# lllllcf/Realtime-Depth-Estimation-Nconv

Hardware: AMD Instinct MI355X
Metric: frames/sec (352x1216 sparse depth, DNET NConv U-Net forward, B=8 per GPU) (higher is better)
Workload: dtype fp32

## Files before the change

### realtime-depth-estimation-nconv_amd/csrc/nconv_fwd_head.hip

```cpp
#include "nconv_prologue.h"

namespace nconv {

namespace {

constexpr int kHT = 256, kHTH = 16, kHTW = 32;
constexpr int kSH = kHTH + 8, kSW = kHTW + 8;
constexpr int kHH = kHTH + 4, kHW = kHTW + 4;
constexpr int kHP = kHW - 16;
constexpr int kHPlane = kHH * kHP;
constexpr int kHPS = kHPlane + 1;
constexpr int kFrag = 2 * 3 * 64 * 4;
constexpr int kLut = 0, kW8R = 4096, kW8C = kW8R + kSH * kSW, kTabEnd = kW8C + kHTH * kSW;
constexpr int kDP = 8 * 64 + 16;
constexpr int kDOff = (kTabEnd + 15) & ~15;

typedef const float __attribute__((address_space(4))) cfloat;
typedef __bf16 bf16x8 __attribute__((ext_vector_type(8)));

template <bool TR>
__global__ __launch_bounds__(kHT) __attribute__((amdgpu_waves_per_eu(5, 8))) void fwd_head_exact(LayerDev d2, TailArgs t, float* __restrict__ y,
                                                      float* __restrict__ yc) {
    const nconv_layer& L = d2.L;
    __shared__ __attribute__((aligned(16))) float sx[kSH * kSW];
    __shared__ __attribute__((aligned(16))) f2 hp[8 * kHPS];
    __shared__ __attribute__((aligned(16))) float w1t[25 * 8];
    __shared__ unsigned long long rowmask[kSH];
    __shared__ unsigned long long c0row[kSH];
    __shared__ unsigned c0col[kSW];
    __shared__ int tile_nan;
    static_assert(kDOff + 8 * kDP * 4 <= (int)sizeof(hp), "D2 tables and transpose fit the plane region");
    const int tid = threadIdx.x;
    const int H = L.Ho, W = L.Wo;
    const TileCoord tc = xcd_tile((W + kHTW - 1) / kHTW, (H + kHTH - 1) / kHTH, L.B);
    const int b = tc.b, R0 = tc.ty * kHTH, C0 = tc.tx * kHTW;
    const bool interior = R0 >= 2 && R0 + kHTH + 2 <= H && C0 >= 2 && C0 + kHTW + 2 <= W;

    if (tid < kSH) rowmask[tid] = c0row[tid] = 0ull;
    if (tid < kSW) c0col[tid] = 0u;
    if (tid == 0) tile_nan = 0;
    if (tid < 200) w1t[tid] = t.w1[(tid & 7) * 25 + (tid >> 3)];
    __syncthreads();
    {
        const __amdgpu_buffer_rsrc_t rs = plane_rsrc(t.s_in + (size_t)b * H * W, H * W * 4);
        constexpr int NE = (kSH * kSW + kHT - 1) / kHT;
        float sv[NE];
#pragma unroll
        for (int k = 0; k < NE; ++k) {
            const int e = tid + kHT * k, r = e / kSW, c = e - (e / kSW) * kSW;
            const int gr = R0 - 4 + r, gc = C0 - 4 + c;
            const bool in = e < kSH * kSW && (unsigned)gr < (unsigned)H && (unsigned)gc < (unsigned)W;
            sv[k] = ld_f32(rs, in ? (unsigned)(gr * W + gc) * 4u : 0x80000000u);
        }
#pragma unroll
        for (int k = 0; k < NE; ++k) {
            const int e = tid + kHT * k, r = e / kSW, c = e - (e / kSW) * kSW;
            if (e < kSH * kSW) {
                const float c0 = sv[k] > t.thresh1 ? 1.0f : 0.0f;
                const float xc = sv[k] * c0;
                sx[e] = xc;
                if (!(xc == 0.f && c0 == 0.f)) atomicOr(&rowmask[r], 1ull << c);
                if (xc != xc) tile_nan = 1;
                if (c0 != 0.f) {
                    atomicOr(&c0row[r], 1ull << c);
                    atomicOr(&c0col[c], 1u << r);
                }
            }
        }
    }
    __syncthreads();

    const int ty = tid >> 4, j = tid & 15;
    f2 accN[8], accD[8];
#pragma unroll
    for (int o = 0; o < 8; ++o) accN[o] = accD[o] = (f2){0.f, 0.f};

    constexpr int NH = (kHH * kHW + kHT - 1) / kHT;
    auto nconv1_pass = [&](bool want_c, auto exact_c0) __attribute__((always_inline)) {
#pragma unroll 1
        for (int k = 0; k < NH; ++k) {
            const int e = tid + kHT * k;
            const int r = e / kHW, c = e - (e / kHW) * kHW;
            const int gr = R0 - 2 + r, gc = C0 - 2 + c;
            const bool valid = e < kHH * kHW;
            const bool in = valid && (unsigned)gr < (unsigned)H && (unsigned)gc < (unsigned)W;
            unsigned m = 0;
#ifndef NCONV_HEAD_PROBE_NO_N1
#pragma unroll
            for (int kh = 0; kh < 5; ++kh) m |= (unsigned)((rowmask[(valid ? r : 0) + kh] >> c) & 31ull) << (5 * kh);
#endif
            m = in ? m : 0u;
            const float* const sxb = sx + r * kSW + c;
            f2 acc[8];
            {
                const bool any = m != 0u;
                const int tp = any ? __builtin_ctz(m) : 0;
                m &= m - 1u;
                const int kh = (tp * 13) >> 6;
                const float xr = sxb[kh * (kSW - 5) + tp];
                const float xc = any ? xr : 0.f;
                const float cv = decltype(exact_c0)::value ? (xc > t.thresh1 ? 1.0f : 0.0f) : 1.0f;
                const f2 v = (f2){xc, any ? cv : 0.f};
                const f4 wa = reinterpret_cast<const f4*>(w1t)[tp * 2], wb = reinterpret_cast<const f4*>(w1t)[tp * 2 + 1];
                const float wv[8] = {wa.x, wa.y, wa.z, wa.w, wb.x, wb.y, wb.z, wb.w};
#pragma unroll
                for (int o = 0; o < 8; ++o) acc[o] = __builtin_elementwise_fma((f2){wv[o], wv[o]}, v, (f2){0.f, 0.f});
            }
            while (m) {
                const int tp = __builtin_ctz(m);
                m &= m - 1;
                const int kh = (tp * 13) >> 6;
                const float xc = sxb[kh * (kSW - 5) + tp];
                const f2 v = (f2){xc, decltype(exact_c0)::value ? (xc > t.thresh1 ? 1.0f : 0.0f) : 1.0f};
                const f4 wa = reinterpret_cast<const f4*>(w1t)[tp * 2], wb = reinterpret_cast<const f4*>(w1t)[tp * 2 + 1];
                const float wv[8] = {wa.x, wa.y, wa.z, wa.w, wb.x, wb.y, wb.z, wb.w};
#pragma unroll
                for (int o = 0; o < 8; ++o) acc[o] = __builtin_elementwise_fma((f2){wv[o], wv[o]}, v, acc[o]);
            }
            const int h0 = (valid && c < kHP) ? (r * kHP + c) * 2 : kHPlane * 2;
            const int h1 = (valid && c >= 16) ? (r * kHP + c - 16) * 2 + 1 : kHPlane * 2 + 1;
            float* const p0 = reinterpret_cast<float*>(hp) + h0;
            float* const p1 = reinterpret_cast<float*>(hp) + h1;
            const unsigned own = (TR && !want_c && in && (unsigned)(r - 2) < (unsigned)kHTH &&
                                  (unsigned)(c - 2) < (unsigned)kHTW) ? (unsigned)(gr * W + gc) * 4u : 0x80000000u;
#pragma unroll
            for (int o = 0; o < 8; ++o) {
                float y1, cc1;
                nconv_epilogue(acc[o].x, acc[o].y, t.eps1, t.b1[o], t.s1[o], y1, cc1);
                if constexpr (TR) {
                    const size_t po1 = ((size_t)b * 8 + o) * H * W;
                    st_f32(plane_rsrc(t.y1 + po1, H * W * 4), own, y1);
                    st_f32(plane_rsrc(t.c1 + po1, H * W * 4), own, cc1);
                }
                const float v = want_c ? cc1 : y1 * cc1;
                p0[o * kHPS * 2] = v;
                p1[o * kHPS * 2] = v;
            }
        }
    };
    auto nconv1_planes = [&](bool want_c) __attribute__((always_inline)) {
        if (tile_nan) nconv1_pass(want_c, std::true_type{});
        else nconv1_pass(want_c, std::false_type{});
    };
    nconv1_planes(false);
    __syncthreads();

    const cfloat* w2t = (const cfloat*)L.waux + kFrag;
    auto sum_planes = [&](f2 (&acc)[8]) __attribute__((always_inline)) {
#pragma unroll 1
        for (int ci = 0; ci < 8; ++ci) {
            const f2* row = hp + ci * kHPS + ty * kHP + j;
            const cfloat* wr = w2t + ci * 200;
#pragma unroll 1
            for (int kh = 0; kh < 5; ++kh, row += kHP, wr += 40) {
                f2 v[5];
#pragma unroll
                for (int kw = 0; kw < 5; ++kw) v[kw] = row[kw];
#pragma unroll
                for (int kw = 0; kw < 5; ++kw)
#pragma unroll
                    for (int o = 0; o < 8; ++o) {
                        const float wv = wr[kw * 8 + o];
                        acc[o] = __builtin_elementwise_fma((f2){wv, wv}, v[kw], acc[o]);
                    }
            }
        }
    };
#ifndef NCONV_HEAD_PROBE_NO_N2
    sum_planes(accN);
#endif
    __syncthreads();
    if (!interior) {
        nconv1_planes(true);
        __syncthreads();
        sum_planes(accD);
    } else {
        unsigned char* const tb = reinterpret_cast<unsigned char*>(hp);
        float* const dt = reinterpret_cast<float*>(tb + kDOff);
        {
            unsigned dq[4];
#pragma unroll
            for (int i = 0; i < 4; ++i)
                dq[i] = ((tid >> (2 * i)) & 1u) * 0x3F80u + ((tid >> (2 * i + 1)) & 1u) * 0x3F800000u;
            reinterpret_cast<uint4*>(tb + kLut)[tid] = make_uint4(dq[0], dq[1], dq[2], dq[3]);
        }
        for (int e = tid; e < kSH * kSW; e += kHT) {
            const int r = e / kSW, c = e - r * kSW;
            tb[kW8R + e] = (unsigned char)(c0row[r] >> c);
            if (r < kHTH) tb[kW8C + e] = c < kHTW ? (unsigned char)(c0col[c + 8] >> r) : 0;
        }
        __syncthreads();
        {
            const int lane = tid & 63, g = lane >> 4, n = lane & 15, w = tid >> 6;
            const uint4* fr = reinterpret_cast<const uint4*>(L.waux) + lane;
            bf16x8 A[2][3];
#pragma unroll
            for (int bb = 0; bb < 2; ++bb)
#pragma unroll
                for (int ks = 0; ks < 3; ++ks) A[bb][ks] = __builtin_bit_cast(bf16x8, fr[(bb * 3 + ks) * 64]);
            const int pb = w * 4 * kSW + n;
            const int o0 = kW8R + g * kSW + pb, o1 = kW8R + (4 + g) * kSW + pb;
            const int o2 = g == 0 ? kW8R + 8 * kSW + pb : (g == 1 ? kW8C + pb : kW8R + 8 * kSW + 8 + pb);
#pragma unroll
            for (int nb = 0; nb < 8; ++nb) {
                const int po = (nb >> 1) * kSW + 16 * (nb & 1);
                const bf16x8 B0 = __builtin_bit_cast(bf16x8, reinterpret_cast<const uint4*>(tb + kLut)[tb[o0 + po]]);
                const bf16x8 B1 = __builtin_bit_cast(bf16x8, reinterpret_cast<const uint4*>(tb + kLut)[tb[o1 + po]]);
                const bf16x8 B2 = __builtin_bit_cast(bf16x8, reinterpret_cast<const uint4*>(tb + kLut)[tb[o2 + po]]);
#pragma unroll
                for (int bb = 0; bb < 2; ++bb) {
                    f4 acc = (f4){0.f, 0.f, 0.f, 0.f};
                    acc = __builtin_amdgcn_mfma_f32_16x16x32_bf16(A[bb][0], B0, acc, 0, 0, 0);
                    acc = __builtin_amdgcn_mfma_f32_16x16x32_bf16(A[bb][1], B1, acc, 0, 0, 0);
                    acc = __builtin_amdgcn_mfma_f32_16x16x32_bf16(A[bb][2], B2, acc, 0, 0, 0);
                    dt[(4 * bb + g) * kDP + (4 * w + (nb >> 1)) * kHTW + 16 * (nb & 1) + n] =
                        (acc.x + acc.y) + acc.z;
                }
            }
        }
        __syncthreads();
#pragma unroll
        for (int o = 0; o < 8; ++o) accD[o] = (f2){dt[o * kDP + ty * kHTW + j], dt[o * kDP + ty * kHTW + j + 16]};
    }

    constexpr unsigned OOB = 0x80000000u;
    const int oh = R0 + ty;
    const size_t plane = (size_t)H * W;
    const int pbytes = (int)(plane * 4);
    const int Hp = H >> 1, Wp = W >> 1;
    const size_t pplane = (size_t)Hp * Wp;
    const int ppbytes = (int)(pplane * 4);
    unsigned so[2], po[2], pcy[2], pcc[2];
    const bool pool_col = ((j & 1) == 0) && (oh >> 1) < Hp;
#pragma unroll
    for (int h = 0; h < 2; ++h) {
        const int ow = C0 + j + 16 * h;
        so[h] = (oh < H && ow < W) ? (unsigned)(oh * W + ow) * 4u : OOB;
        const unsigned pp = (pool_col && (ow >> 1) < Wp) ? (unsigned)((oh >> 1) * Wp + (ow >> 1)) * 4u : OOB;
        po[h] = (ty & 1) == 0 ? pp : OOB;
        pcy[h] = po[h];
        pcc[h] = (ty & 1) ? pp : OOB;
    }
#pragma unroll
    for (int o = 0; o < 8; ++o) {
        float yv[2], cv[2];
        const float s = L.wsum[o], bo = L.bias[o];
#pragma unroll
        for (int h = 0; h < 2; ++h) {
            const float N = h ? accN[o].y : accN[o].x, D = h ? accD[o].y : accD[o].x;
            nconv_epilogue(N, D, L.eps, bo, s, yv[h], cv[h]);
        }
        const size_t ofs = ((size_t)b * 8 + o) * plane;
        const __amdgpu_buffer_rsrc_t ry = plane_rsrc(y + ofs, pbytes), rc = plane_rsrc(yc + ofs, pbytes);
        const size_t pofs = ((size_t)b * 8 + o) * pplane;
        const __amdgpu_buffer_rsrc_t rpy = plane_rsrc(t.py + pofs, ppbytes), rpc = plane_rsrc(t.pc + pofs, ppbytes);
#pragma unroll
        for (int h = 0; h < 2; ++h) {
            st_f32(ry, so[h], yv[h]);
            st_f32(rc, so[h], cv[h]);
#ifdef NCONV_HEAD_PROBE_NO_POOL
            continue;
#endif
            if constexpr (TR) {
                const float yb = shfl_xor16(yv[h]), cb = shfl_xor16(cv[h]);
                const float ya = shfl_xor1(yv[h]), yd = shfl_xor1(yb), ca = shfl_xor1(cv[h]), cd = shfl_xor1(cb);
                int ay, ac;
                st_f32(rpy, po[h], pool4(yv[h], ya, yb, yd, ay));
                st_f32(rpc, po[h], pool4(cv[h], ca, cb, cd, ac));
                st_f32(plane_rsrc((const float*)(t.parg + pofs), ppbytes), po[h],
                       __builtin_bit_cast(float, (unsigned)(ay | (ac << 2))));
            } else {
                const float vm = pair_rows_max(yv[h], cv[h]);
                const float pm = __builtin_elementwise_maximum(vm, shfl_xor1(vm));
                st_f32(rpy, pcy[h], pm);
                st_f32(rpc, pcc[h], pm);
            }
        }
    }
}

__device__ __forceinline__ int frag_slot(int o, int part, int chunk, int j) {
    const int row = 4 * (o & 3) + part, ks = chunk >> 2, g = chunk & 3;
    return (((o >> 2) * 3 + ks) * 64 + g * 16 + row) * 8 + j;
}

constexpr int kHeadUnits = 83;
__device__ __forceinline__ void head_weights_unit(const float* __restrict__ w1, float s1i,
                                                  const float* __restrict__ w2, float* __restrict__ out,
                                                  int blk, int lane) {
    unsigned short* const fb = reinterpret_cast<unsigned short*>(out);
    if (blk == 81) {
        for (int e = lane; e < 1600; e += 64) {
            const int o = e & 7, kk = (e >> 3) % 25, ci = e / 200;
            out[kFrag + e] = w2[(o * 8 + ci) * 25 + kk];
        }
        return;
    }
    if (blk == 82) {
        for (int e = lane; e < kFrag * 2; e += 64) {
            const int j = e & 7, l = (e >> 3) & 63, ks = (e >> 9) % 3;
            const int part = l & 3, chunk = 4 * ks + (l >> 4);
            if (part == 3 || chunk == 11 || (chunk == 10 && j != 0)) fb[e] = 0;
        }
        return;
    }
    const int qh = blk / 9, qw = blk % 9, o = lane >> 3, i = lane & 7;
    double si = 0.0;
#pragma unroll
    for (int kh = 0; kh < 5; ++kh) {
        const int kh1 = qh - kh;
#pragma unroll
        for (int kw = 0; kw < 5; ++kw) {
            const int kw1 = qw - kw;
            const bool v = kh1 >= 0 && kh1 <= 4 && kw1 >= 0 && kw1 <= 4;
            const double a = (double)w2[((o * 8 + i) * 5 + kh) * 5 + kw];
            const double b = (double)w1[v ? (i * 5 + kh1) * 5 + kw1 : 0];
            si = v ? __builtin_fma(a, b, si) : si;
        }
    }
    si /= (double)s1i;
#pragma unroll
    for (int m = 1; m < 8; m <<= 1) si += __shfl_xor(si, m);
    if (i == 0) {
        const float w = (float)si;
        const float hi = __uint_as_float(__float_as_uint(w) & 0xFFFF0000u);
        const float r = w - hi;
        const float mid = __uint_as_float(__float_as_uint(r) & 0xFFFF0000u);
        const float lo = r - mid;
        const int chunk = qw < 8 ? qh : (qh < 8 ? 9 : 10);
        const int j = qw < 8 ? qw : (qh < 8 ? qh : 0);
        fb[frag_slot(o, 0, chunk, j)] = (unsigned short)(__float_as_uint(hi) >> 16);
        fb[frag_slot(o, 1, chunk, j)] = (unsigned short)(__float_as_uint(mid) >> 16);
        fb[frag_slot(o, 2, chunk, j)] = (unsigned short)(__float_as_uint(lo) >> 16);
    }
}

__global__ __launch_bounds__(64) void head_weights(const float* __restrict__ w1, const float* __restrict__ s1,
                                                   const float* __restrict__ w2, float* __restrict__ out) {
    head_weights_unit(w1, s1[threadIdx.x & 7], w2, out, blockIdx.x, threadIdx.x);
}

__global__ __launch_bounds__(kPrepThreads) void weight_prologue(PrepArgs prep, int nprep, const float* __restrict__ w1,
                                                                 const float* __restrict__ w2, float* __restrict__ w21,
                                                                 PhaseArgs ph, int nphase) {
    const int nhead = w21 ? (kHeadUnits + 3) / 4 : 0;
    int blk = blockIdx.x;
    if (blk < nprep) {
        prep_block(prep.w[blk], prep.s[blk], prep.cout[blk], prep.fan_in[blk], 0);
        return;
    }
    blk -= nprep;
    if (blk < nhead) {
        const int lane = threadIdx.x & 63, unit = 4 * blk + (threadIdx.x >> 6);
        if (unit >= kHeadUnits) return;
        float v[8];
#pragma unroll
        for (int r = 0; r < 8; ++r) v[r] = lane < 25 ? w1[r * 25 + lane] : 0.f;
        float s1i = 0.f;
#pragma unroll
        for (int r = 0; r < 8; ++r) {
            float sr = 0.f;
            if (lane < 25) sr += v[r];
#pragma unroll
            for (int m = 32; m > 0; m >>= 1) sr += __shfl_xor(sr, m);
            if ((lane & 7) == r) s1i = sr;
        }
        head_weights_unit(w1, s1i, w2, w21, unit, lane);
        return;
    }
    blk -= nhead;
    if (blk < nphase) phase_block(ph.w[blk], ph.cin[blk], ph.ci0[blk], ph.out[blk]);
}

constexpr int kTrainProThreads = 512, kTrainHeadBlocks = (kHeadUnits + 7) / 8;
__global__ __launch_bounds__(kTrainProThreads) void train_prologue(PrepArgs prep, int nprep, float* w1, float* w2,
                                                               float* s1, float* s2, int sp1, int sp2,
                                                               float* w21, unsigned* sync, TrainPhaseArgs ph,
                                                               int nphase) {
    __shared__ float lw[1800 + 8];
    __shared__ int last;
    const int tid = threadIdx.x, wave = tid >> 6, lane = tid & 63;
    int blk = blockIdx.x;
    if (blk < nprep) {
        if (tid < kPrepThreads) prep_block(prep.w[blk], prep.s[blk], prep.cout[blk], prep.fan_in[blk], prep.softplus[blk]);
        return;
    }
    blk -= nprep;
    if (w21) {
        if (blk < kTrainHeadBlocks) {
            for (int e = tid; e < 1800; e += kTrainProThreads) {
                const bool one = e < 200;
                const float v = one ? w1[e] : w2[e - 200];
                lw[e] = (one ? sp1 : sp2) ? enforce_pos(v) : v;
            }
            __syncthreads();
            {
                const float v = row_sum_wave(lw + wave * 25, 25, lane);
                if (lane == 0) lw[1800 + wave] = v;
            }
            __syncthreads();
            const int u = 8 * blk + wave;
            if (u < kHeadUnits) head_weights_unit(lw, lw[1800 + (lane & 7)], lw + 200, w21, u, lane);
            __syncthreads();
            if (tid == 0) {
                __threadfence();
                last = atomicAdd(sync, 1u) == (unsigned)(kTrainHeadBlocks - 1);
            }
            __syncthreads();
            if (!last) return;
            __threadfence();
            for (int e = tid; e < 1800; e += kTrainProThreads) {
                if (e < 200) {
                    if (sp1) w1[e] = lw[e];
                } else if (sp2) {
                    w2[e - 200] = lw[e];
                }
            }
            if (tid < 8) s1[tid] = lw[1800 + tid];
            {
                const float v = row_sum_wave(lw + 200 + wave * 200, 200, lane);
                if (lane == 0) s2[wave] = v;
            }
            if (tid == 0) atomicExch(sync, 0u);
            return;
        }
        blk -= kTrainHeadBlocks;
    }
    if (blk < nphase && tid < kPrepThreads) {
        float* W = ph.w[blk];
        const int sp = ph.sp[blk];
        for (int e = tid; e < 1152; e += kPrepThreads) lw[e] = sp ? enforce_pos(W[e]) : W[e];
        __syncthreads();
        if (sp)
            for (int e = tid; e < 1152; e += kPrepThreads) W[e] = lw[e];
        for (int o = wave; o < 8; o += kPrepThreads / 64) {
            const float v = row_sum_wave(lw + o * 144, 144, lane);
            if (lane == 0) ph.s[blk][o] = v;
        }
        phase_block(lw, 16, ph.ci0[blk], ph.out[blk]);
        if (float* bx = ph.box[blk])
            for (int e = tid; e < 1024; e += kPrepThreads) bx[e] = box_weight(lw, ph.ci0[blk], e);
    }
}

}

int launch_fwd_head_exact(const LayerDev& d2, const TailArgs& t, float* y, float* yc, hipStream_t st,
                          const char** why) {
    const nconv_layer& L = d2.L;
    dim3 grid(((L.Wo + kHTW - 1) / kHTW) * ((L.Ho + kHTH - 1) / kHTH) * L.B);
    if (t.y1) hipLaunchKernelGGL(fwd_head_exact<true>, grid, dim3(kHT), 0, st, d2, t, y, yc);
    else hipLaunchKernelGGL(fwd_head_exact<false>, grid, dim3(kHT), 0, st, d2, t, y, yc);
    hipError_t e = hipGetLastError();
    if (e != hipSuccess) {
        *why = hipGetErrorString(e);
        return -5;
    }
    return 0;
}

int launch_weight_prologue(int n, float* const* w, const int* cout, const int* fan_in, float* const* s,
                           const float* w1, const float* w2, float* w21, int nphase, const float* const* pw,
                           const int* pcin, const int* pup_first, float* const* pout, hipStream_t st,
                           const char** why) {
    if (n < 0 || n > PrepArgs::kMax || nphase < 0 || nphase > PhaseArgs::kMax) {
        *why = "too many layers for one nconv_weight_prologue launch (max 32 normalisers, 8 phase layers)";
        return -22;
    }
    PrepArgs a{};
    for (int i = 0; i < n; ++i) {
        a.w[i] = w[i];
        a.s[i] = s[i];
        a.cout[i] = cout[i];
        a.fan_in[i] = fan_in[i];
    }
    PhaseArgs p{};
    for (int i = 0; i < nphase; ++i) {
        p.w[i] = pw[i];
        p.out[i] = pout[i];
        p.ci0[i] = pup_first[i];
        p.cin[i] = pcin[i];
    }
    const int blocks = n + (w21 ? (kHeadUnits + 3) / 4 : 0) + nphase;
    if (blocks == 0) return 0;
    hipLaunchKernelGGL(weight_prologue, dim3(blocks), dim3(kPrepThreads), 0, st, a, n, w1, w2, w21, p, nphase);
    hipError_t e = hipGetLastError();
    if (e != hipSuccess) {
        *why = hipGetErrorString(e);
        return -5;
    }
    return 0;
}

int launch_head_weights(const float* w1, const float* s1, const float* w2, float* out, hipStream_t st,
                        const char** why) {
    hipLaunchKernelGGL(head_weights, dim3(kHeadUnits), dim3(64), 0, st, w1, s1, w2, out);
    hipError_t e = hipGetLastError();
    if (e != hipSuccess) {
        *why = hipGetErrorString(e);
        return -5;
    }
    return 0;
}

int launch_train_prologue(int n, float* const* w, const int* cout, const int* fan_in, const int* sp,
                          float* const* s, int head1, int head2, float* w21, unsigned* sync, int nphase,
                          const int* players, const int* pup_first, float* const* pout, float* const* pbox,
                          hipStream_t st, const char** why) {
    if (n < 0 || n > PrepArgs::kMax || nphase < 0 || nphase > TrainPhaseArgs::kMax) {
        *why = "too many layers for one nconv_train_prologue launch (max 32 layers, 8 phase layers)";
        return -22;
    }
    PrepArgs a{};
    TrainPhaseArgs p{};
    int nprep = 0;
    for (int i = 0; i < n; ++i) {
        bool own = w21 && (i == head1 || i == head2);
        for (int k = 0; k < nphase; ++k) own = own || players[k] == i;
        if (own) continue;
        a.w[nprep] = w[i];
        a.s[nprep] = s[i];
        a.cout[nprep] = cout[i];
        a.fan_in[nprep] = fan_in[i];
        a.softplus[nprep] = sp ? sp[i] : 0;
        ++nprep;
    }
    for (int k = 0; k < nphase; ++k) {
        const int i = players[k];
        p.w[k] = w[i];
        p.s[k] = s[i];
        p.out[k] = pout[k];
        p.box[k] = pbox ? pbox[k] : nullptr;
        p.sp[k] = sp ? sp[i] : 0;
        p.ci0[k] = pup_first[k];
    }
    float *w1 = nullptr, *w2 = nullptr, *s1 = nullptr, *s2 = nullptr;
    int sp1 = 0, sp2 = 0;
    if (w21) {
        w1 = w[head1], w2 = w[head2], s1 = s[head1], s2 = s[head2];
        sp1 = sp ? sp[head1] : 0, sp2 = sp ? sp[head2] : 0;
    }
    const int blocks = nprep + (w21 ? kTrainHeadBlocks : 0) + nphase;
    if (blocks == 0) return 0;
    static_assert(kTrainProThreads / 64 == 8, "a wave per nconv1 / nconv2 row");
    hipLaunchKernelGGL(train_prologue, dim3(blocks), dim3(kTrainProThreads), 0, st, a, nprep, w1, w2, s1, s2, sp1, sp2,
                       w21, sync, p, nphase);
    hipError_t e = hipGetLastError();
    if (e != hipSuccess) {
        *why = hipGetErrorString(e);
        return -5;
    }
    return 0;
}

}
```

Measured before the change: 16580.

## Halve head-kernel plane LDS and hold upper channels in registers for more occupancy

The shared plane buffer shrinks from 8 to 4 channels. Channels 4-7 of the first NConv layer are kept in per-thread registers and written to LDS only after the first half has been summed. The D2 octet tables move into the depth tile buffer and the MFMA transpose runs in two halves, which lets the occupancy hint rise from 5 to 7 waves per EU. The change also adds packed FMA inline asm that takes paired scalar weights, and a scalar-only accumulation path for the confidence pass. In exchange it adds extra barriers and register pressure.

```diff
diff --git a/realtime-depth-estimation-nconv_amd/csrc/nconv_fwd_head.hip b/realtime-depth-estimation-nconv_amd/csrc/nconv_fwd_head.hip
--- a/realtime-depth-estimation-nconv_amd/csrc/nconv_fwd_head.hip
+++ b/realtime-depth-estimation-nconv_amd/csrc/nconv_fwd_head.hip
@@ -11,25 +11,38 @@
 constexpr int kHPlane = kHH * kHP;
 constexpr int kHPS = kHPlane + 1;
 constexpr int kFrag = 2 * 3 * 64 * 4;
-constexpr int kLut = 0, kW8R = 4096, kW8C = kW8R + kSH * kSW, kTabEnd = kW8C + kHTH * kSW;
+constexpr int kPl = 4;
+constexpr int kLut = 0, kDOff = 4096;
+constexpr int kW8R = 0, kW8C = kW8R + kSH * kSW, kTabEnd = kW8C + kHTH * kSW;
 constexpr int kDP = 8 * 64 + 16;
-constexpr int kDOff = (kTabEnd + 15) & ~15;
 
 typedef const float __attribute__((address_space(4))) cfloat;
+typedef const f2 __attribute__((address_space(4))) cf2;
 typedef __bf16 bf16x8 __attribute__((ext_vector_type(8)));
 
+__device__ __forceinline__ void pk_fma_lo(f2& acc, f2 w, f2 v) {
+    asm("v_pk_fma_f32 %0, %1, %2, %0 op_sel_hi:[0,1,1]" : "+v"(acc) : "s"(w), "v"(v));
+}
+__device__ __forceinline__ void pk_fma_hi(f2& acc, f2 w, f2 v) {
+    asm("v_pk_fma_f32 %0, %1, %2, %0 op_sel:[1,0,0]" : "+v"(acc) : "s"(w), "v"(v));
+}
+
 template <bool TR>
-__global__ __launch_bounds__(kHT) __attribute__((amdgpu_waves_per_eu(5, 8))) void fwd_head_exact(LayerDev d2, TailArgs t, float* __restrict__ y,
+__global__ __launch_bounds__(kHT) __attribute__((amdgpu_waves_per_eu(7, 8))) void fwd_head_exact(LayerDev d2, TailArgs t, float* __restrict__ y,
                                                       float* __restrict__ yc) {
     const nconv_layer& L = d2.L;
     __shared__ __attribute__((aligned(16))) float sx[kSH * kSW];
-    __shared__ __attribute__((aligned(16))) f2 hp[8 * kHPS];
+    __shared__ __attribute__((aligned(16))) f2 hp[kPl * kHPS];
     __shared__ __attribute__((aligned(16))) float w1t[25 * 8];
     __shared__ unsigned long long rowmask[kSH];
     __shared__ unsigned long long c0row[kSH];
     __shared__ unsigned c0col[kSW];
     __shared__ int tile_nan;
-    static_assert(kDOff + 8 * kDP * 4 <= (int)sizeof(hp), "D2 tables and transpose fit the plane region");
+    static_assert(kDOff >= kLut + 256 * 16 && kDOff % 16 == 0 && kDOff + kPl * kDP * 4 <= (int)sizeof(hp),
+                  "D2's octet table and one half's transpose fit the plane region");
+    static_assert(kTabEnd <= (int)sizeof(sx), "D2's row / column octet tables fit the depth tile");
+    static_assert(sizeof(sx) + sizeof(hp) + sizeof(w1t) + sizeof(rowmask) + sizeof(c0row) + sizeof(c0col) + 16 <=
+                      160 * 1024 / 7, "seven workgroups per CU");
     const int tid = threadIdx.x;
     const int H = L.Ho, W = L.Wo;
     const TileCoord tc = xcd_tile((W + kHTW - 1) / kHTW, (H + kHTH - 1) / kHTH, L.B);
@@ -76,7 +89,24 @@
     for (int o = 0; o < 8; ++o) accN[o] = accD[o] = (f2){0.f, 0.f};
 
     constexpr int NH = (kHH * kHW + kHT - 1) / kHT;
-    auto nconv1_pass = [&](bool want_c, auto exact_c0) __attribute__((always_inline)) {
+    auto plane_slots = [&](int e, float*& p0, float*& p1) __attribute__((always_inline)) {
+        const int r = e / kHW, c = e - (e / kHW) * kHW;
+        const bool valid = e < kHH * kHW;
+        p0 = reinterpret_cast<float*>(hp) + ((valid && c < kHP) ? (r * kHP + c) * 2 : kHPlane * 2);
+        p1 = reinterpret_cast<float*>(hp) + ((valid && c >= 16) ? (r * kHP + c - 16) * 2 + 1 : kHPlane * 2 + 1);
+    };
+    float held[NH][4];
+#pragma unroll
+    for (int k = 0; k < NH; ++k)
+#pragma unroll
+        for (int o = 0; o < 4; ++o) held[k][o] = 0.f;
+    auto nconv1_pass = [&](auto want_c, auto exact_c0) __attribute__((always_inline)) {
+        constexpr bool WC = decltype(want_c)::value;
+        using acc_t = std::conditional_t<WC, float, f2>;
+        auto fma_w = [](float w, f2 v, acc_t a) __attribute__((always_inline)) -> acc_t {
+            if constexpr (WC) return __builtin_fmaf(w, v.y, a);
+            else return __builtin_elementwise_fma((f2){w, w}, v, a);
+        };
 #pragma unroll 1
         for (int k = 0; k < NH; ++k) {
             const int e = tid + kHT * k;
@@ -91,7 +121,7 @@
 #endif
             m = in ? m : 0u;
             const float* const sxb = sx + r * kSW + c;
-            f2 acc[8];
+            acc_t acc[8];
             {
                 const bool any = m != 0u;
                 const int tp = any ? __builtin_ctz(m) : 0;
@@ -104,7 +134,7 @@
                 const f4 wa = reinterpret_cast<const f4*>(w1t)[tp * 2], wb = reinterpret_cast<const f4*>(w1t)[tp * 2 + 1];
                 const float wv[8] = {wa.x, wa.y, wa.z, wa.w, wb.x, wb.y, wb.z, wb.w};
 #pragma unroll
-                for (int o = 0; o < 8; ++o) acc[o] = __builtin_elementwise_fma((f2){wv[o], wv[o]}, v, (f2){0.f, 0.f});
+                for (int o = 0; o < 8; ++o) acc[o] = fma_w(wv[o], v, acc_t{});
             }
             while (m) {
                 const int tp = __builtin_ctz(m);
@@ -115,67 +145,97 @@
                 const f4 wa = reinterpret_cast<const f4*>(w1t)[tp * 2], wb = reinterpret_cast<const f4*>(w1t)[tp * 2 + 1];
                 const float wv[8] = {wa.x, wa.y, wa.z, wa.w, wb.x, wb.y, wb.z, wb.w};
 #pragma unroll
-                for (int o = 0; o < 8; ++o) acc[o] = __builtin_elementwise_fma((f2){wv[o], wv[o]}, v, acc[o]);
-            }
-            const int h0 = (valid && c < kHP) ? (r * kHP + c) * 2 : kHPlane * 2;
-            const int h1 = (valid && c >= 16) ? (r * kHP + c - 16) * 2 + 1 : kHPlane * 2 + 1;
-            float* const p0 = reinterpret_cast<float*>(hp) + h0;
-            float* const p1 = reinterpret_cast<float*>(hp) + h1;
-            const unsigned own = (TR && !want_c && in && (unsigned)(r - 2) < (unsigned)kHTH &&
+                for (int o = 0; o < 8; ++o) acc[o] = fma_w(wv[o], v, acc[o]);
+            }
+            float *p0, *p1;
+            plane_slots(e, p0, p1);
+#pragma unroll
+            for (int q = NH - 1; q > 0; --q)
+#pragma unroll
+                for (int o = 0; o < 4; ++o) held[q][o] = held[q - 1][o];
+            const unsigned own = (TR && !WC && in && (unsigned)(r - 2) < (unsigned)kHTH &&
                                   (unsigned)(c - 2) < (unsigned)kHTW) ? (unsigned)(gr * W + gc) * 4u : 0x80000000u;
 #pragma unroll
             for (int o = 0; o < 8; ++o) {
                 float y1, cc1;
-                nconv_epilogue(acc[o].x, acc[o].y, t.eps1, t.b1[o], t.s1[o], y1, cc1);
-                if constexpr (TR) {
-                    const size_t po1 = ((size_t)b * 8 + o) * H * W;
+                if constexpr (WC) nconv_epilogue(0.f, acc[o], t.eps1, t.b1[o], t.s1[o], y1, cc1);
+                else nconv_epilogue(acc[o].x, acc[o].y, t.eps1, t.b1[o], t.s1[o], y1, cc1);
+                if constexpr (TR && !WC) {
+                    size_t po1 = ((size_t)b * 8 + o) * H * W;
+                    asm volatile("" : "+s"(po1));
                     st_f32(plane_rsrc(t.y1 + po1, H * W * 4), own, y1);
                     st_f32(plane_rsrc(t.c1 + po1, H * W * 4), own, cc1);
                 }
-                const float v = want_c ? cc1 : y1 * cc1;
-                p0[o * kHPS * 2] = v;
-                p1[o * kHPS * 2] = v;
+                const float v = WC ? cc1 : y1 * cc1;
+                if (o < kPl) {
+                    p0[o * kHPS * 2] = v;
+                    p1[o * kHPS * 2] = v;
+                } else {
+                    held[0][o - kPl] = v;
+                }
             }
         }
     };
-    auto nconv1_planes = [&](bool want_c) __attribute__((always_inline)) {
+    auto store_held = [&]() __attribute__((always_inline)) {
+#pragma unroll
+        for (int k = 0; k < NH; ++k) {
+            float *p0, *p1;
+            plane_slots(tid + kHT * k, p0, p1);
+#pragma unroll
+            for (int o = 0; o < kPl; ++o) {
+                p0[o * kHPS * 2] = held[NH - 1 - k][o];
+                p1[o * kHPS * 2] = held[NH - 1 - k][o];
+            }
+        }
+    };
+    auto nconv1_planes = [&](auto want_c) __attribute__((always_inline)) {
         if (tile_nan) nconv1_pass(want_c, std::true_type{});
         else nconv1_pass(want_c, std::false_type{});
     };
-    nconv1_planes(false);
-    __syncthreads();
+    nconv1_planes(std::false_type{});
 
     const cfloat* w2t = (const cfloat*)L.waux + kFrag;
-    auto sum_planes = [&](f2 (&acc)[8]) __attribute__((always_inline)) {
+    auto sum_planes = [&](f2 (&acc)[8], int ci0) __attribute__((always_inline)) {
 #pragma unroll 1
-        for (int ci = 0; ci < 8; ++ci) {
+        for (int ci = 0; ci < kPl; ++ci) {
             const f2* row = hp + ci * kHPS + ty * kHP + j;
-            const cfloat* wr = w2t + ci * 200;
+            const cf2* wr = reinterpret_cast<const cf2*>(w2t + (ci0 + ci) * 200);
 #pragma unroll 1
-            for (int kh = 0; kh < 5; ++kh, row += kHP, wr += 40) {
+            for (int kh = 0; kh < 5; ++kh, row += kHP, wr += 20) {
                 f2 v[5];
 #pragma unroll
                 for (int kw = 0; kw < 5; ++kw) v[kw] = row[kw];
 #pragma unroll
                 for (int kw = 0; kw < 5; ++kw)
 #pragma unroll
-                    for (int o = 0; o < 8; ++o) {
-                        const float wv = wr[kw * 8 + o];
-                        acc[o] = __builtin_elementwise_fma((f2){wv, wv}, v[kw], acc[o]);
+                    for (int o = 0; o < 8; o += 2) {
+                        const f2 wv = wr[kw * 4 + (o >> 1)];
+                        pk_fma_lo(acc[o], wv, v[kw]);
+                        pk_fma_hi(acc[o + 1], wv, v[kw]);
                     }
             }
         }
+    };
+    auto sum_halves = [&](f2 (&acc)[8]) __attribute__((always_inline)) {
+        __syncthreads();
+        sum_planes(acc, 0);
+        __syncthreads();
+        store_held();
+        __syncthreads();
+        sum_planes(acc, kPl);
+        __syncthreads();
     };
 #ifndef NCONV_HEAD_PROBE_NO_N2
-    sum_planes(accN);
+    sum_halves(accN);
+#else
+    __syncthreads();
 #endif
-    __syncthreads();
     if (!interior) {
-        nconv1_planes(true);
-        __syncthreads();
-        sum_planes(accD);
+        nconv1_planes(std::true_type{});
+        sum_halves(accD);
     } else {
         unsigned char* const tb = reinterpret_cast<unsigned char*>(hp);
+        unsigned char* const ob = reinterpret_cast<unsigned char*>(sx);
         float* const dt = reinterpret_cast<float*>(tb + kDOff);
         {
             unsigned dq[4];
@@ -186,41 +246,39 @@
         }
         for (int e = tid; e < kSH * kSW; e += kHT) {
             const int r = e / kSW, c = e - r * kSW;
-            tb[kW8R + e] = (unsigned char)(c0row[r] >> c);
-            if (r < kHTH) tb[kW8C + e] = c < kHTW ? (unsigned char)(c0col[c + 8] >> r) : 0;
+            ob[kW8R + e] = (unsigned char)(c0row[r] >> c);
+            if (r < kHTH) ob[kW8C + e] = c < kHTW ? (unsigned char)(c0col[c + 8] >> r) : 0;
         }
         __syncthreads();
-        {
-            const int lane = tid & 63, g = lane >> 4, n = lane & 15, w = tid >> 6;
-            const uint4* fr = reinterpret_cast<const uint4*>(L.waux) + lane;
-            bf16x8 A[2][3];
-#pragma unroll
-            for (int bb = 0; bb < 2; ++bb)
-#pragma unroll
-                for (int ks = 0; ks < 3; ++ks) A[bb][ks] = __builtin_bit_cast(bf16x8, fr[(bb * 3 + ks) * 64]);
-            const int pb = w * 4 * kSW + n;
-            const int o0 = kW8R + g * kSW + pb, o1 = kW8R + (4 + g) * kSW + pb;
-            const int o2 = g == 0 ? kW8R + 8 * kSW + pb : (g == 1 ? kW8C + pb : kW8R + 8 * kSW + 8 + pb);
+        const int lane = tid & 63, g = lane >> 4, n = lane & 15, w = tid >> 6;
+        const uint4* fr = reinterpret_cast<const uint4*>(L.waux) + lane;
+        const int pb = w * 4 * kSW + n;
+        const int o0 = kW8R + g * kSW + pb, o1 = kW8R + (4 + g) * kSW + pb;
+        const int o2 = g == 0 ? kW8R + 8 * kSW + pb : (g == 1 ? kW8C + pb : kW8R + 8 * kSW + 8 + pb);
+#pragma unroll
+        for (int bb = 0; bb < 2; ++bb) {
+            bf16x8 A[3];
+#pragma unroll
+            for (int ks = 0; ks < 3; ++ks) A[ks] = __builtin_bit_cast(bf16x8, fr[(bb * 3 + ks) * 64]);
+            if (bb) __syncthreads();
 #pragma unroll
             for (int nb = 0; nb < 8; ++nb) {
                 const int po = (nb >> 1) * kSW + 16 * (nb & 1);
-                const bf16x8 B0 = __builtin_bit_cast(bf16x8, reinterpret_cast<const uint4*>(tb + kLut)[tb[o0 + po]]);
-                const bf16x8 B1 = __builtin_bit_cast(bf16x8, reinterpret_cast<const uint4*>(tb + kLut)[tb[o1 + po]]);
-                const bf16x8 B2 = __builtin_bit_cast(bf16x8, reinterpret_cast<const uint4*>(tb + kLut)[tb[o2 + po]]);
-#pragma unroll
-                for (int bb = 0; bb < 2; ++bb) {
-                    f4 acc = (f4){0.f, 0.f, 0.f, 0.f};
-                    acc = __builtin_amdgcn_mfma_f32_16x16x32_bf16(A[bb][0], B0, acc, 0, 0, 0);
-                    acc = __builtin_amdgcn_mfma_f32_16x16x32_bf16(A[bb][1], B1, acc, 0, 0, 0);
-                    acc = __builtin_amdgcn_mfma_f32_16x16x32_bf16(A[bb][2], B2, acc, 0, 0, 0);
-                    dt[(4 * bb + g) * kDP + (4 * w + (nb >> 1)) * kHTW + 16 * (nb & 1) + n] =
-                        (acc.x + acc.y) + acc.z;
-                }
-            }
-        }
-        __syncthreads();
-#pragma unroll
-        for (int o = 0; o < 8; ++o) accD[o] = (f2){dt[o * kDP + ty * kHTW + j], dt[o * kDP + ty * kHTW + j + 16]};
+                const bf16x8 B0 = __builtin_bit_cast(bf16x8, reinterpret_cast<const uint4*>(tb + kLut)[ob[o0 + po]]);
+                const bf16x8 B1 = __builtin_bit_cast(bf16x8, reinterpret_cast<const uint4*>(tb + kLut)[ob[o1 + po]]);
+                const bf16x8 B2 = __builtin_bit_cast(bf16x8, reinterpret_cast<const uint4*>(tb + kLut)[ob[o2 + po]]);
+                f4 acc = (f4){0.f, 0.f, 0.f, 0.f};
+                acc = __builtin_amdgcn_mfma_f32_16x16x32_bf16(A[0], B0, acc, 0, 0, 0);
+                acc = __builtin_amdgcn_mfma_f32_16x16x32_bf16(A[1], B1, acc, 0, 0, 0);
+                acc = __builtin_amdgcn_mfma_f32_16x16x32_bf16(A[2], B2, acc, 0, 0, 0);
+                dt[g * kDP + (4 * w + (nb >> 1)) * kHTW + 16 * (nb & 1) + n] =
+                    (acc.x + acc.y) + acc.z;
+            }
+            __syncthreads();
+#pragma unroll
+            for (int o = 0; o < kPl; ++o)
+                accD[kPl * bb + o] = (f2){dt[o * kDP + ty * kHTW + j], dt[o * kDP + ty * kHTW + j + 16]};
+        }
     }
 
     constexpr unsigned OOB = 0x80000000u;
```

Measured after the change: 16430. No clear change (-0.9%).
